# CompVis/unsupervised-part-segmentation

Measured on AMD Instinct MI355X. Metric: images/sec training (CUB 128x128, 10 parts), higher is better.
Workload: dtype bf16

## Files before the change

unsupervised-part-segmentation_amd/csrc/conv_aux.hip:

```cpp
#include "common.h"

namespace {

template <typename T>
__global__ void weight_prep_kernel(const float* __restrict__ src, int ntaps, int cin_v, int ci_log, int co,
                                   T* __restrict__ wf, int ci_pad, T* __restrict__ wd, int drows, int dk) {
    constexpr int BK = 64 / (int)sizeof(T);
    const int kcf = (ci_pad + BK - 1) / BK, kcd = (dk + BK - 1) / BK;
    const long long nf = wf ? (long long)ntaps * kcf * co * BK : 0;
    const long long nd = wd ? (long long)ntaps * kcd * drows * BK : 0;
    for (long long idx = (long long)blockIdx.x * blockDim.x + threadIdx.x; idx < nf + nd;
         idx += (long long)gridDim.x * blockDim.x) {
        if (idx < nf) {
            const int kk = (int)(idx % BK);
            long long t = idx / BK;
            const int c = (int)(t % co); t /= co;
            const int kc = (int)(t % kcf), tap = (int)(t / kcf);
            const int k = kc * BK + kk;
            const float v = k < ci_log ? src[((long long)tap * cin_v + k) * co + c] : 0.f;
            st_from_float<T>(wf + idx, v);
        } else {
            const long long j = idx - nf;
            const int kk = (int)(j % BK);
            long long t = j / BK;
// ... 152 lines not shown
                    const int e = q * 256 + threadIdx.x;
                    st_from_float<T>(dst + e, tile4[e & 31][e >> 5]);
                }
                j += 3;
                continue;
            }
        }
        weight_prep_chunk<T>(it, c0i * 256, tile);
    }
}

struct Taps3 { int dy[3], dx[3]; };

__global__ void coord_table_kernel(const float* __restrict__ V, int kh, int kw, int ci_log, int co, Taps3 tp, int in_sy,
                                   int in_sx, float ax, float ay, float* __restrict__ tab) {
    const int cls = blockIdx.y;
    const int ym = cls >> 3, xm = cls & 7;
    const int c = blockIdx.x * blockDim.x + threadIdx.x;
    if (c >= co) return;
    float k0, kj, ki;
    coord_table_entry(V, kh, kw, ci_log + 2, ci_log, co, c, ym, xm, tp.dy, tp.dx, in_sy, in_sx, ax, ay, k0, kj, ki);
    tab[((long long)cls * 3 + 0) * co + c] = k0;
    tab[((long long)cls * 3 + 1) * co + c] = kj;
    tab[((long long)cls * 3 + 2) * co + c] = ki;
}

template <typename T>
__global__ void batch_sum_kernel(const T* __restrict__ d, int n, long long pix, int co, int ldo, float* __restrict__ g) {
    constexpr int E = Chunk<T>::N;
    const int cpr = (co + E - 1) / E;
    const long long total = pix * cpr;
    for (long long idx = (long long)blockIdx.x * blockDim.x + threadIdx.x; idx < total;
         idx += (long long)gridDim.x * blockDim.x) {
        const int k = (int)(idx % cpr);
        const long long px = idx / cpr;
        float acc[E];
#pragma unroll
        for (int e = 0; e < E; ++e) acc[e] = 0.f;
        const T* base = d + px * ldo + k * E;
#pragma unroll 4
        for (int b = 0; b < n; ++b) {
            float f[E];
            const uint4 u = *(const uint4*)(base + (long long)b * pix * ldo);
            Chunk<T>::unpack(u, f);
#pragma unroll
            for (int e = 0; e < E; ++e) acc[e] += f[e];
        }
#pragma unroll
        for (int e = 0; e < E; ++e)
            if (k * E + e < co) g[px * co + k * E + e] = acc[e];
    }
}

__global__ __launch_bounds__(256) void coord_rows_kernel(const float* __restrict__ g, int hi, int ho, int wo, int co, int kh, Taps3 tp,
                                                         int in_sy, float ay, float* __restrict__ scratch) {
    __shared__ float red[8][7][32];
    const int o = threadIdx.x & 31, grp = threadIdx.x >> 5;
    const long long plane = (long long)wo * co;
    const long long idx = (long long)blockIdx.x * 32 + o;
    const bool ok = idx < plane;
    float A[4] = {0.f, 0.f, 0.f, 0.f}, B[3] = {0.f, 0.f, 0.f};
    if (ok) {
#pragma unroll 4
        for (int i = grp; i < ho; i += 8) {
            const float v = g[(long long)i * plane + idx];
#pragma unroll
            for (int r = 0; r < 3; ++r) {
                if (r < kh) {
                    const int y = i * in_sy + (r == 0 ? tp.dy[0] : (r == 1 ? tp.dy[1] : tp.dy[2]));
                    if ((unsigned)y < (unsigned)hi) { A[r] += v; B[r] += (ay * (float)y - 1.f) * v; }
                }
            }
            A[3] += v;
        }
    }
#pragma unroll
    for (int r = 0; r < 3; ++r) { red[grp][2 * r][o] = A[r]; red[grp][2 * r + 1][o] = B[r]; }
    red[grp][6][o] = A[3];
    __syncthreads();
    if (grp == 0 && ok) {
#pragma unroll
        for (int q = 0; q < 7; ++q) {
            float t = red[0][q][o];
#pragma unroll
            for (int k = 1; k < 8; ++k) t += red[k][q][o];
            if (q < 6) { if ((q >> 1) < kh) scratch[(long long)q * plane + idx] = t; }
            else scratch[(2 * kh) * plane + idx] = t;
        }
    }
}

__global__ __launch_bounds__(256) void coord_cols_kernel(const float* __restrict__ scratch, int wi, int wo, int co, int kh, int kw, Taps3 tp,
                                                         int in_sx, float ax, int ci_log, float* __restrict__ gV, float* __restrict__ gb) {
    __shared__ float red[4][2][64];
    const int cl = threadIdx.x & 63, grp = threadIdx.x >> 6;
    const int c = blockIdx.x * 64 + cl;
    const int tap = blockIdx.y;
    const long long plane = (long long)wo * co;
    const bool ok = c < co;
    float sx = 0.f, sy = 0.f;
    if (tap == kh * kw) {
        if (!gb) return;
        if (ok) {
#pragma unroll 4
            for (int j = grp; j < wo; j += 4) sx += scratch[(2 * kh) * plane + (long long)j * co + c];
        }
// ... 149 lines not shown
                                   int32_t C, void* w, void* stream) {
    UPS_CHECK_ARG(src && w && ci_log >= 1 && cin_v >= ci_log && co >= 1 && C >= ci_log && C >= 8 && (C & (C - 1)) == 0);
    const int kc = (co + 31) / 32;
    const long long total = 9ll * kc * 4 * C * 4;
    hipLaunchKernelGGL(weight_prep_d2s_kernel, dim3((unsigned)((total + 255) / 256)), dim3(256), 0, (hipStream_t)stream, src, cin_v,
                       ci_log, co, pad_y, pad_x, C, kc, (uint4*)w, total);
    UPS_LAUNCH_CHECK();
    return UPS_OK;
}

extern "C" int64_t ups_prep_item_blocks(const ups_prep_item* item_host, int32_t dtype) {
    if (!item_host) return -1;
    return (prep_elems(*item_host, dtype == UPS_F32 ? 16 : 32) + 255) / 256;
}

extern "C" int ups_weight_prep_batch(const ups_prep_item* items, const int64_t* block_prefix, int32_t n_items,
                                     int64_t total_blocks, int32_t dtype, void* stream) {
    UPS_CHECK_ARG(items && block_prefix && n_items >= 1 && total_blocks >= 1 && total_blocks < 0x7fffffffLL);
    if (dtype == UPS_F32)
        hipLaunchKernelGGL(weight_prep_batch_kernel<float>, dim3((unsigned)ups_cdiv(total_blocks, PREP_CPB)), dim3(256), 0, (hipStream_t)stream,
                           items, (const long long*)block_prefix, n_items, (long long)total_blocks);
    else if (dtype == UPS_F16)
        hipLaunchKernelGGL(weight_prep_batch_kernel<f16>, dim3((unsigned)ups_cdiv(total_blocks, PREP_CPB)), dim3(256), 0, (hipStream_t)stream,
                           items, (const long long*)block_prefix, n_items, (long long)total_blocks);
    else
        hipLaunchKernelGGL(weight_prep_batch_kernel<bf16>, dim3((unsigned)ups_cdiv(total_blocks, PREP_CPB)), dim3(256), 0, (hipStream_t)stream,
                           items, (const long long*)block_prefix, n_items, (long long)total_blocks);
    UPS_LAUNCH_CHECK();
    return UPS_OK;
}

static Taps3 make_taps3(int kh, int kw, const int32_t* dy, const int32_t* dx) {
    Taps3 t;
    for (int i = 0; i < 3; ++i) { t.dy[i] = 0; t.dx[i] = 0; }
    for (int r = 0; r < kh; ++r) t.dy[r] = dy[r * kw];
    for (int s = 0; s < kw; ++s) t.dx[s] = dx[s];
    return t;
}

extern "C" int ups_coord_table(const float* V, int32_t kh, int32_t kw, int32_t ci_log, int32_t co, const int32_t* tap_dy,
                               const int32_t* tap_dx, int32_t in_sy, int32_t in_sx, float ax, float ay, float* tab,
                               void* stream) {
    UPS_CHECK_ARG(V && tab && tap_dy && tap_dx && kh >= 1 && kh <= 3 && kw >= 1 && kw <= 3);
    hipLaunchKernelGGL(coord_table_kernel, dim3(ups_cdiv(co, 128), 64), dim3(128), 0, (hipStream_t)stream, V, kh, kw,
                       ci_log, co, make_taps3(kh, kw, tap_dy, tap_dx), in_sy, in_sx, ax, ay, tab);
    UPS_LAUNCH_CHECK();
    return UPS_OK;
}

extern "C" int ups_batch_sum(const void* dout, int32_t dtype, int32_t n, int64_t pix, int32_t co, int32_t ldo, float* gsum,
                             void* stream) {
    UPS_CHECK_ARG(dout && gsum && n > 0 && pix > 0);
    UPS_CHECK_ARG(ldo % 8 == 0 && ((uintptr_t)dout & 15) == 0);
    int grid = ups_cdiv(pix * ups_cdiv(co, dtype == UPS_F32 ? 4 : 8), 256);
    if (grid > 16384) grid = 16384;
    if (dtype == UPS_F32)
        hipLaunchKernelGGL(batch_sum_kernel<float>, dim3(grid), dim3(256), 0, (hipStream_t)stream, (const float*)dout, n,
                           (long long)pix, co, ldo, gsum);
    else
        hipLaunchKernelGGL(batch_sum_kernel<bf16>, dim3(grid), dim3(256), 0, (hipStream_t)stream, (const bf16*)dout, n,
                           (long long)pix, co, ldo, gsum);
    UPS_LAUNCH_CHECK();
    return UPS_OK;
}

extern "C" int ups_coord_wgrad(const float* gsum, int32_t hi, int32_t wi, int32_t ho, int32_t wo, int32_t co, int32_t kh,
                               int32_t kw, const int32_t* tap_dy, const int32_t* tap_dx, int32_t in_sy, int32_t in_sx,
                               float ax, float ay, int32_t ci_log, float* gradV, float* grad_bias, float* scratch,
                               void* stream) {
    UPS_CHECK_ARG(gsum && gradV && scratch && kh >= 1 && kh <= 3 && kw >= 1 && kw <= 3);
    const Taps3 tp = make_taps3(kh, kw, tap_dy, tap_dx);
    hipStream_t s = (hipStream_t)stream;
    hipLaunchKernelGGL(coord_rows_kernel, dim3(ups_cdiv((long long)wo * co, 32)), dim3(256), 0, s, gsum, hi, ho, wo, co, kh,
                       tp, in_sy, ay, scratch);
    UPS_LAUNCH_CHECK();
    hipLaunchKernelGGL(coord_cols_kernel, dim3(ups_cdiv(co, 64), kh * kw + 1), dim3(256), 0, s, scratch, wi, wo, co, kh, kw,
                       tp, in_sx, ax, ci_log, gradV, grad_bias);
    UPS_LAUNCH_CHECK();
    return UPS_OK;
}

extern "C" int ups_col_sum(const void* dout, int32_t dtype, int64_t rows, int32_t co, int32_t ldo, float* out,
                           float* workspace, void* stream) {
    UPS_CHECK_ARG(dout && out && workspace && rows > 0 && co > 0);
    int tx = 32;
    while (tx < co && tx < 256) tx *= 2;
    const int ty = 256 / tx;
    int nb = (int)((rows + (long long)ty * 16 - 1) / ((long long)ty * 16));
    if (nb > 1024) nb = 1024;
    if (nb < 1) nb = 1;
    hipStream_t s = (hipStream_t)stream;
    if (dtype == UPS_F32)
        hipLaunchKernelGGL(col_sum_kernel<float>, dim3(ups_cdiv(co, tx), nb), dim3(256), 0, s, (const float*)dout,
                           (long long)rows, co, ldo, tx, workspace);
    else
        hipLaunchKernelGGL(col_sum_kernel<bf16>, dim3(ups_cdiv(co, tx), nb), dim3(256), 0, s, (const bf16*)dout,
                           (long long)rows, co, ldo, tx, workspace);
    UPS_LAUNCH_CHECK();
    hipLaunchKernelGGL(col_sum_final_kernel, dim3(ups_cdiv(co, 256)), dim3(256), 0, s, workspace, nb, co, out);
    UPS_LAUNCH_CHECK();
    return UPS_OK;
}
```

unsupervised-part-segmentation_amd/csrc/conv_wgrad3x3.hip:

```cpp
#include <stdlib.h>

#include "common.h"

namespace {

constexpr int TW = 16;
constexpr int PWID = TW + 2;

struct Wg3K {
    int n, h, w, ci, ldi, ci_log, cin_v, co, ldo, act_in, want_bias, units_total, units_per, tiles_x, tiles_y;
    float act_slope;
    unsigned long long tap_off, tap_wi;
    const void* in; const void* dout; float* ws;
    const unsigned* mask; int mask_B;
    int in_f16;
    int taps_std;
};

__device__ inline int g_dy(unsigned long long off, int t) { return (int)((off >> (4 * t + 2)) & 3) - 1; }
__device__ inline int g_dx(unsigned long long off, int t) { return (int)((off >> (4 * t)) & 3) - 1; }
__device__ inline int g_w(unsigned long long wi, int t) { return (int)((wi >> (4 * t)) & 15); }

constexpr int lds_stride3(int row_bytes) { return ((row_bytes + 63) / 128) * 128 + 64; }

typedef __attribute__((address_space(3))) s16x4 lds3_s16x4;

__device__ inline bf16x8 tr_frag3(const unsigned char* tile, int rs, int row0, int c0, int lane) {
    const int g = lane >> 4, i = lane & 15, h = g >> 1;
    const int cb = c0 + 16 * (g & 1), q = i >> 2, pp = i & 3;
    const unsigned char* a0 = tile + (row0 + 8 * h + q) * rs + (cb + 4 * pp) * 2;
    s16x4 lo = __builtin_amdgcn_ds_read_tr16_b64_v4i16((lds3_s16x4*)a0);
    s16x4 hi = __builtin_amdgcn_ds_read_tr16_b64_v4i16((lds3_s16x4*)(a0 + 4 * rs));
    union { s16x4 s[2]; bf16x8 b; } u;
    u.s[0] = lo; u.s[1] = hi;
    return u.b;
}

template <int BN> __device__ __forceinline__ int d_swz(int row) {
    if constexpr (BN == 128) return row & 3;
    else if constexpr (BN == 64) return (row >> 1) & 1;
    else return 0;
}

template <int BN>
__device__ inline bf16x8 tr_frag_d(const unsigned char* tile, int row0, int wco, int lane) {
    constexpr int RS = BN * 2;
    const int g = lane >> 4, i = lane & 15, h = g >> 1, q = i >> 2, pp = i & 3;
    const int row = row0 + 8 * h + q;
    const unsigned char* a0 = tile + row * RS + ((wco ^ d_swz<BN>(row)) << 6) + 32 * (g & 1) + 8 * pp;
    s16x4 lo = __builtin_amdgcn_ds_read_tr16_b64_v4i16((lds3_s16x4*)a0);
    s16x4 hi = __builtin_amdgcn_ds_read_tr16_b64_v4i16((lds3_s16x4*)(a0 + 4 * RS));
    union { s16x4 s[2]; bf16x8 b; } u;
    u.s[0] = lo; u.s[1] = hi;
    return u.b;
}

template <int CB, int BN, int TH, bool SLIDE = false>
__global__ __launch_bounds__(512) void conv_wgrad3x3_kernel(const Wg3K p, const int cit, const int cot, const int nsplit) {
    constexpr int PROWS = TH + 2, PPIX = PWID * PROWS;
    constexpr int WCI = CB / 32, WCO = BN / 32, WK = 8 / (WCI * WCO);
    constexpr int RSX = lds_stride3(CB * 2), RSD = BN * 2;
    constexpr int XB = PPIX * RSX, DB = TH * TW * RSD;
    constexpr int CPX = CB / 8, CPD = BN / 8;
    constexpr int NX = (PPIX * CPX + 511) / 512;
    constexpr int NWD = TH * TW * CPD / 512;
    static_assert(NX <= 3 && NWD >= 1, "staging layout");

    extern __shared__ __attribute__((aligned(16))) unsigned char smem[];
    unsigned char* Xbuf = smem;
    unsigned char* Dbuf = smem + 2 * XB;

    const int tid = threadIdx.x, lane = tid & 63;
    const int wid = __builtin_amdgcn_readfirstlane(tid >> 6);
    const float act_ns = ups_slope_eff(p.act_in, p.act_slope);
    const int pairs = cit * cot;
    int pair = blockIdx.x % pairs, split = blockIdx.x / pairs;
    if ((nsplit & 7) == 0) {
        const int j = blockIdx.x >> 3;
        pair = j % pairs;
        split = (j / pairs) * 8 + (blockIdx.x & 7);
    }
    const int cot_i = pair % cot, cit_i = pair / cot;
    const int w_ci = wid % WCI, w_co = (wid / WCI) % WCO, w_k = wid / (WCI * WCO);
    const int ci0 = cit_i * CB, co0 = cot_i * BN;
    const bf16* __restrict__ in = (const bf16*)p.in;
    const bf16* __restrict__ dout = (const bf16*)p.dout;
    const bool do_bias = p.want_bias && cit_i == 0 && w_ci == 0;

    const int u_begin = split * p.units_per;
    const int u_end = min(p.units_total, u_begin + p.units_per);

    unsigned xr[NX], xs[NX];
#pragma unroll
    for (int k = 0; k < NX; ++k) {
        const int item = min(tid + 512 * k, PPIX * CPX - 1);
        const int pix = item / CPX, cc = item - pix * CPX;
        const int py = pix / PWID, px = pix - py * PWID;
        unsigned fl = (py == 0 ? 1u : 0u) | (py == PROWS - 1 ? 2u : 0u) | (px == 0 ? 4u : 0u) | (px == PWID - 1 ? 8u : 0u);
        if (tid + 512 * k >= PPIX * CPX || ci0 + cc * 8 >= p.ci) fl |= 16u;
        xr[k] = (unsigned)(py * p.w + px);
        xs[k] = (unsigned)(pix * RSX + cc * 16) | (fl << 16);
    }
    const unsigned x_rowb = (unsigned)p.ldi * 2u;
    const unsigned x_chb = (unsigned)(ci0 + (tid % CPX) * 8) * 2u;
    unsigned dd[NWD];
#pragma unroll
    for (int q = 0; q < NWD; ++q) {
        const int L = (wid + 8 * q) * 64 + lane, row = L / CPD, sl = L - row * CPD;
        const int c = sl ^ (d_swz<BN>(row) << 2);
        const int ch = min(co0 + c * 8, p.ldo - 8);
        dd[q] = (unsigned)((((row >> 4) * p.w + (row & 15)) * p.ldo + ch) * 2);
    }
    const unsigned smem_lds = (unsigned)(unsigned long long)(__attribute__((address_space(3))) unsigned char*)smem;

    uint4 rx[NX];
    uint4 rxn[NX];
    bool rxok[NX];
    const uint4 zero4 = make_uint4(0u, 0u, 0u, 0u);

    auto unit_origin = [&](int u, int& img, int& y0, int& x0) {
        const int half = TH == 8 ? (u & 1) : 0;
        int t = TH == 8 ? (u >> 1) : u;
        const int tx = t % p.tiles_x; t /= p.tiles_x;
        const int ty = t % p.tiles_y;
        img = t / p.tiles_y;
        y0 = ty * 16 + half * TH; x0 = tx * TW;
    };
    auto load_x = [&](int u) __attribute__((always_inline)) {
        int img, y0, x0;
        unit_origin(u, img, y0, x0);
        const unsigned edge = (y0 == 0 ? 1u : 0u) | (y0 + TH == p.h ? 2u : 0u) | (x0 == 0 ? 4u : 0u) | (x0 + TW == p.w ? 8u : 0u) | 16u;
        const long long org = ((long long)img * p.h + (y0 - 1)) * p.w + (x0 - 1);
        const unsigned char* xb = (const unsigned char*)(in + org * p.ldi);
#pragma unroll
        for (int k = 0; k < NX; ++k) {
            unsigned r = xr[k], f = xs[k];
            asm volatile("" : "+v"(r), "+v"(f));
            const bool ok = ((f >> 16) & edge) == 0u;
            const unsigned char* src = ok ? xb + (__umul24(r, x_rowb) + x_chb) : (const unsigned char*)in;
            uint4 v;
            asm volatile("global_load_dwordx4 %0, %1, off" : "=v"(v) : "v"(src) : "memory");
            rxn[k] = v;
            rxok[k] = ok;
        }
    };
    auto dma_d = [&](int u, int buf) __attribute__((always_inline)) {
        int img, y0, x0;
        unit_origin(u, img, y0, x0);
        const unsigned char* db = (const unsigned char*)(dout + (((long long)img * p.h + y0) * p.w + x0) * p.ldo);
#pragma unroll
        for (int q = 0; q < NWD; ++q) {
            const unsigned lds_dst = __builtin_amdgcn_readfirstlane(smem_lds + (unsigned)(2 * XB + buf * DB + (wid + 8 * q) * 1024));
            asm volatile("s_mov_b32 m0, %0\n\ts_nop 0\n\tglobal_load_lds_dwordx4 %1, %2"
                         :: "s"(lds_dst), "v"(dd[q]), "s"(db) : "memory", "m0");
        }
    };
    auto store_xn = [&](int buf) __attribute__((always_inline)) {
        unsigned char* X = Xbuf + buf * XB;
#pragma unroll
        for (int k = 0; k < NX; ++k) {
            unsigned f = xs[k];
            asm volatile("" : "+v"(f));
            uint4 v = rxok[k] ? rxn[k] : zero4;
            if (p.in_f16) v = ups_act_chunk_f16_to_bf16(v, act_ns, p.act_in != UPS_ACT_NONE);
            else if (p.act_in != UPS_ACT_NONE) v = ups_act_chunk(v, act_ns, (bf16*)nullptr);
            if (k + 1 < NX || tid + 512 * k < PPIX * CPX) *(uint4*)(X + (f & 0xffffu)) = v;
            __builtin_amdgcn_sched_barrier(0);
        }
    };
    auto load_unit = [&](int u, int buf) __attribute__((always_inline)) {
        int img, y0, x0;
        unit_origin(u, img, y0, x0);
        const unsigned edge = (y0 == 0 ? 1u : 0u) | (y0 + TH == p.h ? 2u : 0u) | (x0 == 0 ? 4u : 0u) | (x0 + TW == p.w ? 8u : 0u) | 16u;
        const int img_x = p.mask ? img % p.mask_B : img;
        const int part = p.mask ? img / p.mask_B : 0;
        const long long org = ((long long)img_x * p.h + (y0 - 1)) * p.w + (x0 - 1);
        const unsigned char* xb = (const unsigned char*)(in + org * p.ldi);
        const unsigned* mb = p.mask ? p.mask + org : nullptr;
#pragma unroll
        for (int k = 0; k < NX; ++k) {
            unsigned r = xr[k], f = xs[k];
            asm volatile("" : "+v"(r), "+v"(f));
            uint4 v = zero4;
            if (((f >> 16) & edge) == 0u) {
                v = *(const uint4*)(xb + (__umul24(r, x_rowb) + x_chb));
                if (mb && !((mb[r] >> part) & 1u)) v = zero4;
            }
            rx[k] = v;
        }
        const unsigned char* db = (const unsigned char*)(dout + (((long long)img * p.h + y0) * p.w + x0) * p.ldo);
#pragma unroll
        for (int q = 0; q < NWD; ++q) {
            const unsigned lds_dst = __builtin_amdgcn_readfirstlane(smem_lds + (unsigned)(2 * XB + buf * DB + (wid + 8 * q) * 1024));
            asm volatile("s_mov_b32 m0, %0\n\ts_nop 0\n\tglobal_load_lds_dwordx4 %1, %2"
                         :: "s"(lds_dst), "v"(dd[q]), "s"(db) : "memory", "m0");
        }
    };
    auto store_unit = [&](int buf) __attribute__((always_inline)) {
        unsigned char* X = Xbuf + buf * XB;
#pragma unroll
        for (int k = 0; k < NX; ++k) {
            unsigned f = xs[k];
            asm volatile("" : "+v"(f));
            uint4 v = rx[k];
            if (p.in_f16) v = ups_act_chunk_f16_to_bf16(v, act_ns, p.act_in != UPS_ACT_NONE);
            else if (p.act_in != UPS_ACT_NONE) v = ups_act_chunk(v, act_ns, (bf16*)nullptr);
            if (k + 1 < NX || tid + 512 * k < PPIX * CPX) *(uint4*)(X + (f & 0xffffu)) = v;
            __builtin_amdgcn_sched_barrier(0);
        }
    };

    f32x16 acc[9];
#pragma unroll
    for (int t = 0; t < 9; ++t)
#pragma unroll
        for (int e = 0; e < 16; ++e) acc[t][e] = 0.f;
    float bsum = 0.f;

    if constexpr (WK == 1 && SLIDE) {
      if (!p.mask) {
        static_assert(NX == 3 && (NWD == 4 || NWD == 2 || NWD == 1), "pipelined staging: item / DMA piece counts");
#define UPS_WAIT_X(N) asm volatile("s_waitcnt vmcnt(" #N ")" : "+v"(rxn[0].x), "+v"(rxn[0].y), "+v"(rxn[0].z), "+v"(rxn[0].w), \
                                   "+v"(rxn[1].x), "+v"(rxn[1].y), "+v"(rxn[1].z), "+v"(rxn[1].w), "+v"(rxn[2].x), "+v"(rxn[2].y), \
// ... 4 lines not shown
            store_xn(0);
            if (u_begin + 1 < u_end) load_x(u_begin + 1);
        }
        UPS_WAIT_X(0);
        __syncthreads();
        for (int u = u_begin; u < u_end; ++u) {
            const int buf = (u - u_begin) & 1;
            if (u + 1 < u_end) dma_d(u + 1, buf ^ 1);
            const unsigned char* X = Xbuf + buf * XB;
            const unsigned char* D = Dbuf + buf * DB;
            bf16x8 aw[3][3];
#pragma unroll
            for (int dxi = 0; dxi < 3; ++dxi) {
                aw[0][dxi] = tr_frag3(X, RSX, dxi, w_ci * 32, lane);
                aw[1][dxi] = tr_frag3(X, RSX, PWID + dxi, w_ci * 32, lane);
            }
            bf16x8 bcur = tr_frag_d<BN>(D, 0, w_co, lane);
#pragma unroll
            for (int ks = 0; ks < TH; ++ks) {
                if (ks == TH / 2) {
                    if (u + 1 < u_end) {
                        if (NWD == 4) UPS_WAIT_X(4); else if (NWD == 2) UPS_WAIT_X(2); else UPS_WAIT_X(1);
                        store_xn(buf ^ 1);
                    }
                    if (u + 2 < u_end) load_x(u + 2);
                    __builtin_amdgcn_sched_barrier(0);
                }
#pragma unroll
                for (int dxi = 0; dxi < 3; ++dxi) aw[(ks + 2) % 3][dxi] = tr_frag3(X, RSX, (ks + 2) * PWID + dxi, w_ci * 32, lane);
                const bf16x8 bnext = tr_frag_d<BN>(D, (ks + 1 < TH ? ks + 1 : ks) * TW, w_co, lane);
                const bf16x8 b = bcur;
#pragma unroll
                for (int t = 0; t < 9; ++t)
                    acc[t] = __builtin_amdgcn_mfma_f32_32x32x16_bf16(aw[(ks + t / 3) % 3][t % 3], b, acc[t], 0, 0, 0);
                if (do_bias) {
#pragma unroll
                    for (int j = 0; j < 8; ++j) bsum += (float)b[j];
                }
                bcur = bnext;
                __builtin_amdgcn_sched_barrier(0);
            }
            if (u + 2 < u_end) {
                if (NX == 3) asm volatile("s_waitcnt vmcnt(3)" ::: "memory");
                else asm volatile("s_waitcnt vmcnt(2)" ::: "memory");
            } else {
                asm volatile("s_waitcnt vmcnt(0)" ::: "memory");
            }
            asm volatile("s_waitcnt lgkmcnt(0)" ::: "memory");
            __builtin_amdgcn_s_barrier();
        }
        goto reduce_parts;
      }
    }
    if (u_begin < u_end) { load_unit(u_begin, 0); store_unit(0); }
    asm volatile("s_waitcnt vmcnt(0)" ::: "memory");
    __syncthreads();
    for (int u = u_begin; u < u_end; ++u) {
        const int buf = (u - u_begin) & 1;
        if (u + 1 < u_end) load_unit(u + 1, buf ^ 1);
        const unsigned char* X = Xbuf + buf * XB;
        const unsigned char* D = Dbuf + buf * DB;
        if constexpr (WK == 1 && SLIDE) {
            bf16x8 aw[3][3];
#pragma unroll
            for (int dxi = 0; dxi < 3; ++dxi) {
                aw[0][dxi] = tr_frag3(X, RSX, dxi, w_ci * 32, lane);
                aw[1][dxi] = tr_frag3(X, RSX, PWID + dxi, w_ci * 32, lane);
            }
#pragma unroll
            for (int ks = 0; ks < TH; ++ks) {
#pragma unroll
                for (int dxi = 0; dxi < 3; ++dxi) aw[(ks + 2) % 3][dxi] = tr_frag3(X, RSX, (ks + 2) * PWID + dxi, w_ci * 32, lane);
                const bf16x8 b = tr_frag_d<BN>(D, ks * TW, w_co, lane);
#pragma unroll
                for (int t = 0; t < 9; ++t)
                    acc[t] = __builtin_amdgcn_mfma_f32_32x32x16_bf16(aw[(ks + t / 3) % 3][t % 3], b, acc[t], 0, 0, 0);
                if (do_bias) {
#pragma unroll
                    for (int j = 0; j < 8; ++j) bsum += (float)b[j];
                }
                __builtin_amdgcn_sched_barrier(0);
            }
        } else
#pragma unroll 1
        for (int kk = 0; kk < TH / WK; ++kk) {
            const int ks = w_k + kk * WK;
            const bf16x8 b = tr_frag_d<BN>(D, ks * TW, w_co, lane);
#pragma unroll
            for (int t = 0; t < 9; ++t) {
                const int row0 = SLIDE ? (ks + t / 3) * PWID + t % 3 : (ks + g_dy(p.tap_off, t) + 1) * PWID + g_dx(p.tap_off, t) + 1;
                const bf16x8 a = tr_frag3(X, RSX, row0, w_ci * 32, lane);
                acc[t] = __builtin_amdgcn_mfma_f32_32x32x16_bf16(a, b, acc[t], 0, 0, 0);
            }
            if (do_bias) {
#pragma unroll
                for (int j = 0; j < 8; ++j) bsum += (float)b[j];
            }
        }
        if (u + 1 < u_end) store_unit(buf ^ 1);
        asm volatile("s_waitcnt vmcnt(0)" ::: "memory");
        __syncthreads();
    }

reduce_parts:
    bsum += __shfl_xor(bsum, 32, 64);
    if (WK > 1) {
        float* red = (float*)smem;
        const int slot = ((w_k - 1) * (WCI * WCO) + w_ci + WCI * w_co) * 1024;
        const int slot0 = (w_ci + WCI * w_co) * 1024;
#pragma unroll
        for (int t = 0; t < 9; ++t) {
            __syncthreads();
            if (w_k > 0) {
#pragma unroll
                for (int e = 0; e < 16; ++e) red[slot + e * 64 + lane] = acc[t][e];
            }
            __syncthreads();
            if (w_k == 0) {
                for (int k = 1; k < WK; ++k)
#pragma unroll
                    for (int e = 0; e < 16; ++e) acc[t][e] += red[(k - 1) * (WCI * WCO) * 1024 + slot0 + e * 64 + lane];
            }
        }
        __syncthreads();
        if (w_k > 0) red[slot + lane] = bsum;
        __syncthreads();
        if (w_k == 0)
            for (int k = 1; k < WK; ++k) bsum += red[(k - 1) * (WCI * WCO) * 1024 + slot0 + lane];
    }
    const long long slab_sz = (long long)9 * p.cin_v * p.co + p.co;
    float* slab = p.ws + (long long)split * slab_sz;
    const int col = co0 + w_co * 32 + (lane & 31);
    if (w_k == 0 && col < p.co) {
#pragma unroll
        for (int t = 0; t < 9; ++t) {
            const int tw = g_w(p.tap_wi, t);
#pragma unroll
            for (int e = 0; e < 16; ++e) {
                const int row = ci0 + w_ci * 32 + (e & 3) + 8 * (e >> 2) + 4 * (lane >> 5);
                if (row < p.ci_log) slab[((long long)tw * p.cin_v + row) * p.co + col] = acc[t][e];
            }
        }
        if (do_bias && (lane >> 5) == 0) slab[(long long)9 * p.cin_v * p.co + col] = bsum;
    }
}

struct Variant { int cb, bn, wk, th; };

Variant pick(const ups_wgrad_desc* d) {
    Variant v;
    v.cb = d->ci > 32 ? 64 : 32;
    v.bn = d->co > 64 ? 128 : (d->co > 32 ? 64 : 32);
    v.wk = 8 / ((v.cb / 32) * (v.bn / 32));
    v.th = (v.cb == 32 && v.bn <= 64) ? 16 : 8;
    return v;
}

bool eligible(const ups_wgrad_desc* d) {
    if (d->dtype != UPS_BF16 || d->ntaps != 9 || d->in_sy != 1 || d->in_sx != 1) return false;
    if (d->hi != d->ho || d->wi != d->wo || d->hi % 16 || d->wi % 16) return false;
    if (19ll * d->wi * d->ldi * 2 >= (1ll << 31) || 17ll * d->wi * d->ldo * 2 >= (1ll << 31)) return false;
    if (18ll * d->wi >= (1 << 24) || (long long)d->ldi * 2 >= (1 << 24)) return false;
    bool seen[9] = {false, false, false, false, false, false, false, false, false};
    for (int t = 0; t < 9; ++t) {
        const int dy = d->tap_dy[t], dx = d->tap_dx[t];
        if (dy < -1 || dy > 1 || dx < -1 || dx > 1 || d->tap_w[t] < 0 || d->tap_w[t] > 8) return false;
        seen[(dy + 1) * 3 + dx + 1] = true;
    }
    for (int t = 0; t < 9; ++t) if (!seen[t]) return false;
    return !ups_env_off_now("UPS_FORCE_GENERIC_CONV");
}

template <int CB, int BN, int TH, bool SLIDE = false>
int launch3(const Wg3K& k, int cit, int cot, int splitk, hipStream_t s) {
    constexpr int RSX = lds_stride3(CB * 2), RSD = BN * 2;
    constexpr int PPIX = PWID * (TH + 2);
    size_t shmem = 2 * (size_t)(PPIX * RSX + TH * TW * RSD);
    constexpr size_t red = (size_t)(8 / ((CB / 32) * (BN / 32)) - 1) * (CB / 32) * (BN / 32) * 4096;
    if (shmem < red) shmem = red;
    return ups_launch_lds<conv_wgrad3x3_kernel<CB, BN, TH, SLIDE>>("conv_wgrad3x3_kernel", shmem, dim3(cit * cot * splitk), dim3(512), shmem, s,
                                                                   k, cit, cot, splitk);
}

}

int ups_wgrad3x3_plan(const ups_wgrad_desc* d, int* splitk, int* slabs) {
    if (!eligible(d)) return 1;
    const Variant v = pick(d);
    const int pairs = ups_cdiv(d->ci, v.cb) * ups_cdiv(d->co, v.bn);
    const int units = d->n * (d->hi / 16) * (d->wi / 16) * (16 / v.th);
    int sk = ups_cdiv((v.cb == 64 && v.bn == 128) ? 256 : 512, pairs);
    if (sk > units / 4) sk = units / 4 > 0 ? units / 4 : 1;
    if (sk > 256) sk = 256;
    if (sk >= 8) sk &= ~7;
    *splitk = sk;
    *slabs = sk;
    return 0;
}

int ups_wgrad3x3_run(const ups_wgrad_desc* d, hipStream_t s) {
    const Variant v = pick(d);
    Wg3K k;
    k.n = d->n; k.h = d->hi; k.w = d->wi; k.ci = d->ci; k.ldi = d->ldi; k.ci_log = d->ci_log; k.cin_v = d->cin_v;
    k.co = d->co; k.ldo = d->ldo; k.act_in = d->act_in; k.act_slope = d->act_slope; k.want_bias = d->grad_bias != nullptr;
    k.tiles_x = d->wi / 16; k.tiles_y = d->hi / 16;
    k.units_total = d->n * k.tiles_x * k.tiles_y * (16 / v.th);
    k.units_per = ups_cdiv(k.units_total, d->splitk);
    k.in = d->in; k.dout = d->dout; k.ws = d->workspace;
    k.mask = d->mask_bits; k.mask_B = d->mask_batch;
    k.in_f16 = d->in_f16;
    k.taps_std = 1;
    for (int t = 0; t < 9; ++t) if (d->tap_dy[t] != t / 3 - 1 || d->tap_dx[t] != t % 3 - 1) k.taps_std = 0;
    if (!ups_env_on_now("UPS_WGRAD_SLIDE")) k.taps_std = 0;
    k.tap_off = 0; k.tap_wi = 0;
    for (int t = 0; t < 9; ++t) {
        k.tap_off |= (unsigned long long)(((d->tap_dy[t] + 1) << 2) | (d->tap_dx[t] + 1)) << (4 * t);
        k.tap_wi |= (unsigned long long)d->tap_w[t] << (4 * t);
    }
    const int cit = ups_cdiv(d->ci, v.cb), cot = ups_cdiv(d->co, v.bn);
    if (v.cb == 64 && v.bn == 128) return k.taps_std ? launch3<64, 128, 8, true>(k, cit, cot, d->splitk, s) : launch3<64, 128, 8>(k, cit, cot, d->splitk, s);
    if (v.cb == 64 && v.bn == 64) return k.taps_std ? launch3<64, 64, 8, true>(k, cit, cot, d->splitk, s) : launch3<64, 64, 8>(k, cit, cot, d->splitk, s);
    if (v.cb == 64 && v.bn == 32) return k.taps_std ? launch3<64, 32, 8, true>(k, cit, cot, d->splitk, s) : launch3<64, 32, 8>(k, cit, cot, d->splitk, s);
    if (v.cb == 32 && v.bn == 128) return k.taps_std ? launch3<32, 128, 8, true>(k, cit, cot, d->splitk, s) : launch3<32, 128, 8>(k, cit, cot, d->splitk, s);
    if (v.cb == 32 && v.bn == 64) return k.taps_std ? launch3<32, 64, 16, true>(k, cit, cot, d->splitk, s) : launch3<32, 64, 16>(k, cit, cot, d->splitk, s);
    return k.taps_std ? launch3<32, 32, 16, true>(k, cit, cot, d->splitk, s) : launch3<32, 32, 16>(k, cit, cot, d->splitk, s);
}
```

unsupervised-part-segmentation_amd/switches.py:

```python
import os
from collections import OrderedDict

SWITCHES = OrderedDict([
    ("UPS_LIB", ("", "ab", "lib.py", "path of the library to load instead of csrc/libupsparts_hip.so (A/B builds: tools/ab_build.sh)")),
    ("UPS_DIST_BACKEND", ("nccl", "product", "runner.py", "torch.distributed backend (nccl = RCCL; gloo for the CPU / one-GPU tests)")),
    ("UPS_GRAPH", ("0", "product", "model.py", "1: HIP-graph replay of the step (config key hip_graph)")),
    ("UPS_STREAM_PLAN", ("auto", "product", "model.py", "full | compact | auto: side-stream budget (config key stream_plan; DESIGN section 7)")),
    ("UPS_NO_OVERLAP", ("0", "ab", "ops.py", "1: everything on one stream (per-kernel profiles without CU sharing)")),
    ("UPS_POST_ACT", ("1", "ab", "nets.py", "0: activation-on-load everywhere instead of post-activation storage (config key post_activation_storage)")),
    ("UPS_SIGN_BITS", ("1", "ab", "ops.py", "0: input gradients read the forward input for act' instead of the producer's sign bytes")),
    ("UPS_VGG_FP8", ("0", "ab", "model.py", "1: fp8 copies through the perceptual trunk (config key vgg_fp8; measured slower, DESIGN 3b)")),
    ("UPS_F8_WGRAD", ("1", "ab", "ops.py", "0: bf16 weight gradients in precision fp8")),
    ("UPS_F8_PRODUCER", ("1", "ab", "ops.py", "0: fp8 copies converted by a separate pass instead of the producing epilogue")),
    ("UPS_TOWERS", ("1", "ab", "ops.py", "0: the critics' towers through the generic convolution path instead of the grouped launches")),
    ("UPS_STATE_KERNEL", ("1", "ab", "model.py", "0: the Lagrangian / EMA state update as ~30 torch launches instead of one kernel")),
    ("UPS_LATE_JOIN", ("1", "ab", "stepsync.py", "0: a single rank joins the weight-gradient stream at every segment boundary")),
    ("UPS_EARLY_ADAM", ("1", "ab", "stepsync.py", "0: every key's Adam at the end of the step instead of behind its weight gradients")),
    ("UPS_EARLY_ALPHA", ("1", "ab", "model.py", "0: the appearance code after the pose encoder instead of beside it on `aux`")),
    ("UPS_CRITIC_STREAMS", ("1", "ab", "model.py", "0: the three critics on one stream")),
    ("UPS_COORD_STREAM", ("1", "ab", "ops.py", "0: the CoordConv rows of the weight gradients on the weight-gradient stream itself")),
    ("UPS_NO_D2S", ("0", "ab", "ops.py", "1: the stride-2 layers' input gradient as four phase launches instead of one depth-to-space launch")),
    ("UPS_DP_SIDE_LAUNCH", ("1", "ab", "stepsync.py", "0: bucket all-reduces launched from the launching stream (it then waits for the weight gradients)")),
    ("UPS_DP_STANDIN", ("0", "debug", "dist.py", "1: every bucket all-reduce replaced by a device copy on its own stream (one-GPU stream-budget probe)")),
    ("UPS_FORCE_COLLECTIVES", ("0", "test", "dist.py", "1: issue the collectives at world size 1 (the RCCL call pattern test)")),
    ("UPS_JOIN_TIMING", ("0", "debug", "stepsync.py", "1: HIP events around the end-of-backward joins (tools/probes/join_wait.py)")),
    ("UPS_ROWS_KERNEL", ("1", "test", "conv3x3_rows.hip", "0: row-stream layers through the patch / generic kernels; force: also at small batches (parity tests)")),
    ("UPS_S2_KERNEL", ("1", "ab", "conv3x3_s2.hip", "0: the other stride-2 forwards through the generic kernel")),
    ("UPS_THIN_SW", ("32", "ab", "conv3x3_rows.hip", "16: 16-column strips in the logit convolution (measured equal)")),
    ("UPS_FIRST_LAYER", ("1", "ab", "conv3x3_first.hip", "0: the 3-channel first layers through the generic kernel")),
    ("UPS_FORCE_GENERIC_CONV", ("0", "test", "conv_igemm.hip", "1: every convolution through the generic gather kernel")),
    ("UPS_IGEMM_FORCE", ("", "test", "conv_igemm.hip", "tile variant of the generic kernel")),
    ("UPS_NO_SPLITK", ("0", "ab", "conv_igemm.hip", "1: no split-K for the small-grid generic launches")),
    ("UPS_NO_SMALL_PATCH", ("0", "ab", "conv3x3_patch.hip", "1: no small-tile patch instances")),
    ("UPS_PATCH_CST", ("", "ab", "conv3x3_patch.hip", "patch kernel: constant-stride instances on / off")),
    ("UPS_PATCH_DMA", ("1", "ab", "conv3x3_patch.hip", "0: register-staged patches instead of LDS-DMA")),
    ("UPS_PATCH_MID", ("", "ab", "conv3x3_patch.hip", "patch kernel: mid-size tile selection")),
    ("UPS_PATCH_OCC", ("", "ab", "conv3x3_patch.hip", "patch kernel: blocks per CU override")),
    ("UPS_PATCH_RAGGED", ("1", "ab", "conv3x3_patch.hip", "0: images that are not a multiple of 16 leave the patch kernel")),
    ("UPS_PATCH_STATIC", ("", "ab", "conv3x3_patch.hip", "patch kernel: static-geometry instances on / off")),
    ("UPS_PATCH_THIN128", ("", "ab", "conv3x3_patch.hip", "patch kernel: thin 128-wide instance selection")),
    ("UPS_PATCH_THINOUT", ("", "ab", "conv3x3_patch.hip", "patch kernel: thin-output instance selection")),
    ("UPS_RES_PATCH", ("1", "ab", "conv3x3_patch.hip", "0: the forward's residual from global memory instead of the resident patch")),
    ("UPS_RES_PATCH_DGRAD", ("1", "ab", "conv3x3_patch.hip", "0: the input gradient's residual and sign bytes fetched in the epilogue instead of from the resident patch (round 6)")),
    ("UPS_F8_SCALED", ("1", "ab", "conv3x3_patch.hip", "0: K = 32 fp8 MFMA instead of the block-scaled K = 128 form")),
    ("UPS_WGRAD_DIRECT", ("1", "ab", "conv_wgrad.hip", "0: single-split weight gradients through a slab + reduce launch")),
    ("UPS_WGRAD_SLIDE", ("1", "ab", "conv_wgrad3x3.hip", "0: the plain form of the 3x3 weight gradient (3 % slower step)")),
    ("UPS_PRIOR_PX", ("1", "ab", "priors.hip", "0: the staged prior kernels at P = 10 instead of the pixel-per-lane rings")),
    ("UPS_PRIOR_PX_BPI", ("", "test", "priors.hip", "cap on blocks per image of the pixel-per-lane prior kernels (multi-tile loops at three images)")),
    ("UPS_PRIOR_DIRECT", ("1", "ab", "priors.hip", "0: the staged prior kernels at P = 16 / 20 / 25 instead of the chunk-per-lane direct-from-global forms (round 6)")),
    ("UPS_SOFTMAX_PX", ("1", "ab", "partpath.hip", "0: the LDS-walking soft-max kernel at P = 10")),
    ("UPS_MOMENTS_PX", ("1", "ab", "partpath.hip", "0: the slab form of the spatial moments at P = 10")),
    ("UPS_MOMENTS_PX_BLOCKS", ("", "test", "partpath.hip", "blocks of the pixel-per-lane moments kernel")),
    ("UPS_UNPOOL_MFMA", ("1", "test", "partpath.hip", "0: the VALU form of unpool_bwd (the unit test compares both)")),
])

COMPILE_TIME = ("UPS_ROWS_FWD_SIGN", "UPS_ROWS_NO_FENCE", "UPS_VMAX_BUILTIN")
NOT_SWITCHES = ("UPS_ABI_VERSION", "UPS_ACT_", "UPS_OK", "UPS_E_", "UPS_BF16", "UPS_F16", "UPS_F32", "UPS_CHECK_ARG", "UPS_LAUNCH_CHECK")


def value(name):
    return os.environ.get(name, SWITCHES[name][0])


def flag(name):
    d = SWITCHES[name][0]
    v = os.environ.get(name, d)
    return v != "0" if d == "1" else v == "1"


def report():
    diff = ["{}={}".format(k, os.environ[k]) for k, (d, _, _, _) in SWITCHES.items() if k in os.environ and os.environ[k] != d]
    return "UPS switches: " + (", ".join(diff) if diff else "all defaults")
```

Baseline: 2106.

## Pack small 8x8/4x4 maps into 128-pixel wgrad units; split batch sums across groups

Adds a packed-image variant of the 3x3 weight-gradient MFMA kernel for 8x8 and 4x4 feature maps. Each unit holds 128 pixels from several images, placed in a zero-padded LDS layout, so these layers no longer fall back to the generic split-K gather kernel. It also adds a batch-sum kernel that splits the batch loop across thread groups with an LDS reduction when the grid would otherwise be small, to raise parallelism. The cost is more template instances, a zeroing pass over LDS, and new indexing paths that could be wrong at edge cases.

```diff
diff --git a/unsupervised-part-segmentation_amd/csrc/conv_aux.hip b/unsupervised-part-segmentation_amd/csrc/conv_aux.hip
--- a/unsupervised-part-segmentation_amd/csrc/conv_aux.hip
+++ b/unsupervised-part-segmentation_amd/csrc/conv_aux.hip
@@ -228,6 +228,54 @@
     }
 }
 
+template <typename T, int G>
+__global__ __launch_bounds__(256) void batch_sum_split_kernel(const T* __restrict__ d, int n, long long pix, int co, int ldo,
+                                                              float* __restrict__ g) {
+    constexpr int E = Chunk<T>::N, OPB = 256 / G;
+    __shared__ float sh[256 * E];
+    const int cpr = (co + E - 1) / E;
+    const long long total = pix * cpr;
+    const int o = threadIdx.x % OPB, gi = threadIdx.x / OPB;
+    const long long idx = (long long)blockIdx.x * OPB + o;
+    const bool valid = idx < total;
+    const int k = valid ? (int)(idx % cpr) : 0;
+    const long long px = valid ? idx / cpr : 0;
+    float acc[E];
+#pragma unroll
+    for (int e = 0; e < E; ++e) acc[e] = 0.f;
+    if (valid) {
+        const T* base = d + px * ldo + k * E;
+#pragma unroll 4
+        for (int b = gi; b < n; b += G) {
+            float f[E];
+            const uint4 u = *(const uint4*)(base + (long long)b * pix * ldo);
+            Chunk<T>::unpack(u, f);
+#pragma unroll
+            for (int e = 0; e < E; ++e) acc[e] += f[e];
+        }
+    }
+    float* mine = sh + (gi * OPB + o) * E;
+#pragma unroll
+    for (int e = 0; e < E; ++e) mine[e] = acc[e];
+    for (int st = G / 2; st >= 1; st >>= 1) {
+        __syncthreads();
+        if (gi < st) {
+            const float* other = sh + ((gi + st) * OPB + o) * E;
+#pragma unroll
+            for (int e = 0; e < E; ++e) acc[e] += other[e];
+            if (st > 1) {
+#pragma unroll
+                for (int e = 0; e < E; ++e) mine[e] = acc[e];
+            }
+        }
+    }
+    if (valid && gi == 0) {
+#pragma unroll
+        for (int e = 0; e < E; ++e)
+            if (k * E + e < co) g[px * co + k * E + e] = acc[e];
+    }
+}
+
 __global__ __launch_bounds__(256) void coord_rows_kernel(const float* __restrict__ g, int hi, int ho, int wo, int co, int kh, Taps3 tp,
                                                          int in_sy, float ay, float* __restrict__ scratch) {
     __shared__ float red[8][7][32];
@@ -483,8 +531,19 @@
                              void* stream) {
     UPS_CHECK_ARG(dout && gsum && n > 0 && pix > 0);
     UPS_CHECK_ARG(ldo % 8 == 0 && ((uintptr_t)dout & 15) == 0);
-    int grid = ups_cdiv(pix * ups_cdiv(co, dtype == UPS_F32 ? 4 : 8), 256);
+    const long long total = pix * ups_cdiv(co, dtype == UPS_F32 ? 4 : 8);
+    int grid = ups_cdiv(total, 256);
     if (grid > 16384) grid = 16384;
+    if (grid < 256 && n > 1 && dtype != UPS_F32) {
+        const int G = total * 4 >= 65536 ? 4 : (total * 16 >= 65536 ? 16 : 64);
+        const hipStream_t s = (hipStream_t)stream;
+        const dim3 sg((unsigned)ups_cdiv(total, 256 / G));
+#define UPS_BSUM_SPLIT(GG) hipLaunchKernelGGL((batch_sum_split_kernel<bf16, GG>), sg, dim3(256), 0, s, (const bf16*)dout, n, (long long)pix, co, ldo, gsum)
+        if (G == 4) UPS_BSUM_SPLIT(4); else if (G == 16) UPS_BSUM_SPLIT(16); else UPS_BSUM_SPLIT(64);
+#undef UPS_BSUM_SPLIT
+        UPS_LAUNCH_CHECK();
+        return UPS_OK;
+    }
     if (dtype == UPS_F32)
         hipLaunchKernelGGL(batch_sum_kernel<float>, dim3(grid), dim3(256), 0, (hipStream_t)stream, (const float*)dout, n,
                            (long long)pix, co, ldo, gsum);
diff --git a/unsupervised-part-segmentation_amd/csrc/conv_wgrad3x3.hip b/unsupervised-part-segmentation_amd/csrc/conv_wgrad3x3.hip
--- a/unsupervised-part-segmentation_amd/csrc/conv_wgrad3x3.hip
+++ b/unsupervised-part-segmentation_amd/csrc/conv_wgrad3x3.hip
@@ -25,12 +25,13 @@
 
 typedef __attribute__((address_space(3))) s16x4 lds3_s16x4;
 
+template <int PH = 8, int PE = 4>
 __device__ inline bf16x8 tr_frag3(const unsigned char* tile, int rs, int row0, int c0, int lane) {
     const int g = lane >> 4, i = lane & 15, h = g >> 1;
     const int cb = c0 + 16 * (g & 1), q = i >> 2, pp = i & 3;
-    const unsigned char* a0 = tile + (row0 + 8 * h + q) * rs + (cb + 4 * pp) * 2;
+    const unsigned char* a0 = tile + (row0 + PH * h + q) * rs + (cb + 4 * pp) * 2;
     s16x4 lo = __builtin_amdgcn_ds_read_tr16_b64_v4i16((lds3_s16x4*)a0);
-    s16x4 hi = __builtin_amdgcn_ds_read_tr16_b64_v4i16((lds3_s16x4*)(a0 + 4 * rs));
+    s16x4 hi = __builtin_amdgcn_ds_read_tr16_b64_v4i16((lds3_s16x4*)(a0 + PE * rs));
     union { s16x4 s[2]; bf16x8 b; } u;
     u.s[0] = lo; u.s[1] = hi;
     return u.b;
@@ -55,14 +56,17 @@
     return u.b;
 }
 
-template <int CB, int BN, int TH, bool SLIDE = false>
+constexpr int sub_ppix(int sub) { return (128 / (sub * sub)) * (sub + 2) * (sub + 2); }
+
+template <int CB, int BN, int TH, bool SLIDE = false, int SUB = 0>
 __global__ __launch_bounds__(512) void conv_wgrad3x3_kernel(const Wg3K p, const int cit, const int cot, const int nsplit) {
-    constexpr int PROWS = TH + 2, PPIX = PWID * PROWS;
+    static_assert(SUB == 0 || ((SUB == 8 || SUB == 4) && TH == 8 && !SLIDE), "packed-image units: 128 pixels, plain tap loop");
+    constexpr int PROWS = TH + 2, PPIX = SUB ? sub_ppix(SUB ? SUB : 8) : PWID * PROWS;
     constexpr int WCI = CB / 32, WCO = BN / 32, WK = 8 / (WCI * WCO);
     constexpr int RSX = lds_stride3(CB * 2), RSD = BN * 2;
     constexpr int XB = PPIX * RSX, DB = TH * TW * RSD;
     constexpr int CPX = CB / 8, CPD = BN / 8;
-    constexpr int NX = (PPIX * CPX + 511) / 512;
+    constexpr int NX = ((SUB ? 128 : PPIX) * CPX + 511) / 512;
     constexpr int NWD = TH * TW * CPD / 512;
     static_assert(NX <= 3 && NWD >= 1, "staging layout");
 
@@ -93,23 +97,34 @@
     unsigned xr[NX], xs[NX];
 #pragma unroll
     for (int k = 0; k < NX; ++k) {
-        const int item = min(tid + 512 * k, PPIX * CPX - 1);
-        const int pix = item / CPX, cc = item - pix * CPX;
-        const int py = pix / PWID, px = pix - py * PWID;
-        unsigned fl = (py == 0 ? 1u : 0u) | (py == PROWS - 1 ? 2u : 0u) | (px == 0 ? 4u : 0u) | (px == PWID - 1 ? 8u : 0u);
-        if (tid + 512 * k >= PPIX * CPX || ci0 + cc * 8 >= p.ci) fl |= 16u;
-        xr[k] = (unsigned)(py * p.w + px);
-        xs[k] = (unsigned)(pix * RSX + cc * 16) | (fl << 16);
+        if constexpr (SUB != 0) {
+            const int item = tid + 512 * k;
+            const int pix = item / CPX, cc = item - pix * CPX;
+            const int img = pix / (SUB * SUB), y = (pix / SUB) % SUB, x = pix % SUB;
+            const int slot = img * (SUB + 2) * (SUB + 2) + (y + 1) * (SUB + 2) + x + 1;
+            xr[k] = (unsigned)pix;
+            xs[k] = (unsigned)(slot * RSX + cc * 16) | ((ci0 + cc * 8 >= p.ci ? 16u : 0u) << 16);
+        } else {
+            const int item = min(tid + 512 * k, PPIX * CPX - 1);
+            const int pix = item / CPX, cc = item - pix * CPX;
+            const int py = pix / PWID, px = pix - py * PWID;
+            unsigned fl = (py == 0 ? 1u : 0u) | (py == PROWS - 1 ? 2u : 0u) | (px == 0 ? 4u : 0u) | (px == PWID - 1 ? 8u : 0u);
+            if (tid + 512 * k >= PPIX * CPX || ci0 + cc * 8 >= p.ci) fl |= 16u;
+            xr[k] = (unsigned)(py * p.w + px);
+            xs[k] = (unsigned)(pix * RSX + cc * 16) | (fl << 16);
+        }
     }
     const unsigned x_rowb = (unsigned)p.ldi * 2u;
     const unsigned x_chb = (unsigned)(ci0 + (tid % CPX) * 8) * 2u;
+    const unsigned x_chb_in = (unsigned)min(ci0 + (tid % CPX) * 8, p.ldi - 8) * 2u;
     unsigned dd[NWD];
 #pragma unroll
     for (int q = 0; q < NWD; ++q) {
         const int L = (wid + 8 * q) * 64 + lane, row = L / CPD, sl = L - row * CPD;
         const int c = sl ^ (d_swz<BN>(row) << 2);
         const int ch = min(co0 + c * 8, p.ldo - 8);
-        dd[q] = (unsigned)((((row >> 4) * p.w + (row & 15)) * p.ldo + ch) * 2);
+        if constexpr (SUB != 0) dd[q] = (unsigned)((row * p.ldo + ch) * 2);
+        else dd[q] = (unsigned)((((row >> 4) * p.w + (row & 15)) * p.ldo + ch) * 2);
     }
     const unsigned smem_lds = (unsigned)(unsigned long long)(__attribute__((address_space(3))) unsigned char*)smem;
 
@@ -169,6 +184,24 @@
         }
     };
     auto load_unit = [&](int u, int buf) __attribute__((always_inline)) {
+        if constexpr (SUB != 0) {
+            const unsigned char* xb = (const unsigned char*)(in + (long long)u * 128 * p.ldi);
+#pragma unroll
+            for (int k = 0; k < NX; ++k) {
+                unsigned r = xr[k], f = xs[k];
+                asm volatile("" : "+v"(r), "+v"(f));
+                const uint4 v = *(const uint4*)(xb + (__umul24(r, x_rowb) + x_chb_in));
+                rx[k] = ((f >> 16) & 16u) == 0u ? v : zero4;
+            }
+            const unsigned char* db = (const unsigned char*)(dout + (long long)u * 128 * p.ldo);
+#pragma unroll
+            for (int q = 0; q < NWD; ++q) {
+                const unsigned lds_dst = __builtin_amdgcn_readfirstlane(smem_lds + (unsigned)(2 * XB + buf * DB + (wid + 8 * q) * 1024));
+                asm volatile("s_mov_b32 m0, %0\n\ts_nop 0\n\tglobal_load_lds_dwordx4 %1, %2"
+                             :: "s"(lds_dst), "v"(dd[q]), "s"(db) : "memory", "m0");
+            }
+            return;
+        }
         int img, y0, x0;
         unit_origin(u, img, y0, x0);
         const unsigned edge = (y0 == 0 ? 1u : 0u) | (y0 + TH == p.h ? 2u : 0u) | (x0 == 0 ? 4u : 0u) | (x0 + TW == p.w ? 8u : 0u) | 16u;
@@ -279,6 +312,10 @@
         goto reduce_parts;
       }
     }
+    if constexpr (SUB != 0) {
+        for (int i = tid; i < 2 * XB / 16; i += 512) ((uint4*)smem)[i] = zero4;
+        __syncthreads();
+    }
     if (u_begin < u_end) { load_unit(u_begin, 0); store_unit(0); }
     asm volatile("s_waitcnt vmcnt(0)" ::: "memory");
     __syncthreads();
@@ -315,9 +352,16 @@
             const bf16x8 b = tr_frag_d<BN>(D, ks * TW, w_co, lane);
 #pragma unroll
             for (int t = 0; t < 9; ++t) {
-                const int row0 = SLIDE ? (ks + t / 3) * PWID + t % 3 : (ks + g_dy(p.tap_off, t) + 1) * PWID + g_dx(p.tap_off, t) + 1;
-                const bf16x8 a = tr_frag3(X, RSX, row0, w_ci * 32, lane);
-                acc[t] = __builtin_amdgcn_mfma_f32_32x32x16_bf16(a, b, acc[t], 0, 0, 0);
+                if constexpr (SUB != 0) {
+                    const int dy = g_dy(p.tap_off, t), dx = g_dx(p.tap_off, t);
+                    const int row0 = SUB == 8 ? (ks >> 2) * 100 + (2 * (ks & 3) + 1 + dy) * 10 + 1 + dx : ks * 36 + (1 + dy) * 6 + 1 + dx;
+                    const bf16x8 a = tr_frag3<(SUB == 8 ? 10 : 12), (SUB == 8 ? 4 : 6)>(X, RSX, row0, w_ci * 32, lane);
+                    acc[t] = __builtin_amdgcn_mfma_f32_32x32x16_bf16(a, b, acc[t], 0, 0, 0);
+                } else {
+                    const int row0 = SLIDE ? (ks + t / 3) * PWID + t % 3 : (ks + g_dy(p.tap_off, t) + 1) * PWID + g_dx(p.tap_off, t) + 1;
+                    const bf16x8 a = tr_frag3(X, RSX, row0, w_ci * 32, lane);
+                    acc[t] = __builtin_amdgcn_mfma_f32_32x32x16_bf16(a, b, acc[t], 0, 0, 0);
+                }
             }
             if (do_bias) {
 #pragma unroll
@@ -372,10 +416,26 @@
     }
 }
 
-struct Variant { int cb, bn, wk, th; };
+struct Variant { int cb, bn, wk, th, sub; };
+
+int small_sub(const ups_wgrad_desc* d) {
+    if (!((d->hi == 8 && d->wi == 8) || (d->hi == 4 && d->wi == 4))) return 0;
+    if (((long long)d->n * d->hi * d->wi) % 128 != 0 || d->mask_bits) return 0;
+    if (ups_env_int_now("UPS_WGRAD_SMALL", 1) == 0) return 0;
+    return d->wi;
+}
 
 Variant pick(const ups_wgrad_desc* d) {
     Variant v;
+    v.sub = small_sub(d);
+    if (v.sub) {
+        v.cb = 64;
+        v.bn = (d->co > 64 && v.sub == 8) ? 128 : 64;
+        if (v.sub == 4 && d->co > 64 && ups_env_int_now("UPS_WGRAD_SMALL", 1) == 2) { v.cb = 32; v.bn = 128; }
+        v.wk = 8 / ((v.cb / 32) * (v.bn / 32));
+        v.th = 8;
+        return v;
+    }
     v.cb = d->ci > 32 ? 64 : 32;
     v.bn = d->co > 64 ? 128 : (d->co > 32 ? 64 : 32);
     v.wk = 8 / ((v.cb / 32) * (v.bn / 32));
@@ -385,9 +445,14 @@
 
 bool eligible(const ups_wgrad_desc* d) {
     if (d->dtype != UPS_BF16 || d->ntaps != 9 || d->in_sy != 1 || d->in_sx != 1) return false;
-    if (d->hi != d->ho || d->wi != d->wo || d->hi % 16 || d->wi % 16) return false;
-    if (19ll * d->wi * d->ldi * 2 >= (1ll << 31) || 17ll * d->wi * d->ldo * 2 >= (1ll << 31)) return false;
-    if (18ll * d->wi >= (1 << 24) || (long long)d->ldi * 2 >= (1 << 24)) return false;
+    if (d->hi != d->ho || d->wi != d->wo) return false;
+    if (small_sub(d)) {
+        if (128ll * d->ldi * 2 >= (1ll << 31) || 128ll * d->ldo * 2 >= (1ll << 31) || (long long)d->ldi * 2 >= (1 << 24)) return false;
+    } else {
+        if (d->hi % 16 || d->wi % 16) return false;
+        if (19ll * d->wi * d->ldi * 2 >= (1ll << 31) || 17ll * d->wi * d->ldo * 2 >= (1ll << 31)) return false;
+        if (18ll * d->wi >= (1 << 24) || (long long)d->ldi * 2 >= (1 << 24)) return false;
+    }
     bool seen[9] = {false, false, false, false, false, false, false, false, false};
     for (int t = 0; t < 9; ++t) {
         const int dy = d->tap_dy[t], dx = d->tap_dx[t];
@@ -398,15 +463,16 @@
     return !ups_env_off_now("UPS_FORCE_GENERIC_CONV");
 }
 
-template <int CB, int BN, int TH, bool SLIDE = false>
+template <int CB, int BN, int TH, bool SLIDE = false, int SUB = 0>
 int launch3(const Wg3K& k, int cit, int cot, int splitk, hipStream_t s) {
     constexpr int RSX = lds_stride3(CB * 2), RSD = BN * 2;
-    constexpr int PPIX = PWID * (TH + 2);
+    constexpr int PPIX = SUB ? sub_ppix(SUB ? SUB : 8) : PWID * (TH + 2);
     size_t shmem = 2 * (size_t)(PPIX * RSX + TH * TW * RSD);
     constexpr size_t red = (size_t)(8 / ((CB / 32) * (BN / 32)) - 1) * (CB / 32) * (BN / 32) * 4096;
     if (shmem < red) shmem = red;
-    return ups_launch_lds<conv_wgrad3x3_kernel<CB, BN, TH, SLIDE>>("conv_wgrad3x3_kernel", shmem, dim3(cit * cot * splitk), dim3(512), shmem, s,
-                                                                   k, cit, cot, splitk);
+    static_assert(2 * (size_t)(PPIX * RSX + TH * TW * RSD) <= 160 * 1024 && red <= 160 * 1024, "LDS of one block");
+    return ups_launch_lds<conv_wgrad3x3_kernel<CB, BN, TH, SLIDE, SUB>>("conv_wgrad3x3_kernel", shmem, dim3(cit * cot * splitk), dim3(512), shmem, s,
+                                                                        k, cit, cot, splitk);
 }
 
 }
@@ -415,7 +481,7 @@
     if (!eligible(d)) return 1;
     const Variant v = pick(d);
     const int pairs = ups_cdiv(d->ci, v.cb) * ups_cdiv(d->co, v.bn);
-    const int units = d->n * (d->hi / 16) * (d->wi / 16) * (16 / v.th);
+    const int units = v.sub ? (int)((long long)d->n * d->hi * d->wi / 128) : d->n * (d->hi / 16) * (d->wi / 16) * (16 / v.th);
     int sk = ups_cdiv((v.cb == 64 && v.bn == 128) ? 256 : 512, pairs);
     if (sk > units / 4) sk = units / 4 > 0 ? units / 4 : 1;
     if (sk > 256) sk = 256;
@@ -432,6 +498,7 @@
     k.co = d->co; k.ldo = d->ldo; k.act_in = d->act_in; k.act_slope = d->act_slope; k.want_bias = d->grad_bias != nullptr;
     k.tiles_x = d->wi / 16; k.tiles_y = d->hi / 16;
     k.units_total = d->n * k.tiles_x * k.tiles_y * (16 / v.th);
+    if (v.sub) k.units_total = (int)((long long)d->n * d->hi * d->wi / 128);
     k.units_per = ups_cdiv(k.units_total, d->splitk);
     k.in = d->in; k.dout = d->dout; k.ws = d->workspace;
     k.mask = d->mask_bits; k.mask_B = d->mask_batch;
@@ -445,6 +512,8 @@
         k.tap_wi |= (unsigned long long)d->tap_w[t] << (4 * t);
     }
     const int cit = ups_cdiv(d->ci, v.cb), cot = ups_cdiv(d->co, v.bn);
+    if (v.sub == 8) return v.bn == 128 ? launch3<64, 128, 8, false, 8>(k, cit, cot, d->splitk, s) : launch3<64, 64, 8, false, 8>(k, cit, cot, d->splitk, s);
+    if (v.sub == 4) return v.cb == 32 ? launch3<32, 128, 8, false, 4>(k, cit, cot, d->splitk, s) : launch3<64, 64, 8, false, 4>(k, cit, cot, d->splitk, s);
     if (v.cb == 64 && v.bn == 128) return k.taps_std ? launch3<64, 128, 8, true>(k, cit, cot, d->splitk, s) : launch3<64, 128, 8>(k, cit, cot, d->splitk, s);
     if (v.cb == 64 && v.bn == 64) return k.taps_std ? launch3<64, 64, 8, true>(k, cit, cot, d->splitk, s) : launch3<64, 64, 8>(k, cit, cot, d->splitk, s);
     if (v.cb == 64 && v.bn == 32) return k.taps_std ? launch3<64, 32, 8, true>(k, cit, cot, d->splitk, s) : launch3<64, 32, 8>(k, cit, cot, d->splitk, s);
diff --git a/unsupervised-part-segmentation_amd/switches.py b/unsupervised-part-segmentation_amd/switches.py
--- a/unsupervised-part-segmentation_amd/switches.py
+++ b/unsupervised-part-segmentation_amd/switches.py
@@ -45,6 +45,7 @@
     ("UPS_F8_SCALED", ("1", "ab", "conv3x3_patch.hip", "0: K = 32 fp8 MFMA instead of the block-scaled K = 128 form")),
     ("UPS_WGRAD_DIRECT", ("1", "ab", "conv_wgrad.hip", "0: single-split weight gradients through a slab + reduce launch")),
     ("UPS_WGRAD_SLIDE", ("1", "ab", "conv_wgrad3x3.hip", "0: the plain form of the 3x3 weight gradient (3 % slower step)")),
+    ("UPS_WGRAD_SMALL", ("1", "ab", "conv_wgrad3x3.hip", "0: the 3x3 weight gradients of 8x8 / 4x4 maps through the generic split-K kernel instead of packed-image units; 2: the <32,128> instance at 4x4 instead of <64,64>")),
     ("UPS_PRIOR_PX", ("1", "ab", "priors.hip", "0: the staged prior kernels at P = 10 instead of the pixel-per-lane rings")),
     ("UPS_PRIOR_PX_BPI", ("", "test", "priors.hip", "cap on blocks per image of the pixel-per-lane prior kernels (multi-tile loops at three images)")),
     ("UPS_PRIOR_DIRECT", ("1", "ab", "priors.hip", "0: the staged prior kernels at P = 16 / 20 / 25 instead of the chunk-per-lane direct-from-global forms (round 6)")),
```

After: 2110 (median of 4 runs). Within noise of the previous version (+0.2%).
